# KevynUtopia/Frequency-Aware-Inverse-Consistent-OCTA-Super-Resolution

Hardware: AMD Instinct MI355X
Metric: train-step images/sec (G+D fwd+bwd) on 256x256 OCTA (higher is better)
Workload: dtype f32 (tensors and accumulators fp32; the convolutions' operands enter the matrix cores as f16x2 pairs: hi = f16(x 2^k), lo = f16(x 2^k - hi), k from the tensor's largest magnitude; 3 v_mfma_f32_32x32x16_f16 per product) on every map >= 24 wide with >= 16 channels; narrow maps, 1-channel stems / head

## Files before the change

### frequency-aware-inverse-consistent-octa-super-resolution_amd/csrc/common.h

```cpp
#pragma once
#include <hip/hip_runtime.h>
#include <cstdio>
#include <cstdarg>
#include "faoctasr.h"

namespace faoctasr {

char* err_buf();
int fail(int code, const char* fmt, ...);
enum Route { ROUTE_NONE = 0, ROUTE_GATHER_FLAT = 1, ROUTE_PATCH = 2, ROUTE_WINOGRAD = 3, ROUTE_BF16X3 = 4, ROUTE_M1_FWD = 5, ROUTE_NARROW = 6,
             ROUTE_WGRAD_FLAT = 11, ROUTE_WGRAD_PATCH = 12, ROUTE_WGRAD_S1 = 13, ROUTE_M1_WGRAD = 14, ROUTE_WGRAD_X3 = 15, ROUTE_STEM_DGRAD = 7, ROUTE_STEM_WGRAD = 16,
             ROUTE_NARROW_X2 = 8 };
void set_route(int r);
extern thread_local int g_no_split_k;
extern thread_local unsigned* g_out_absmax;
unsigned* take_out_absmax();

void lds_optin(const void* kernel, size_t lds_bytes);

inline int check_launch(const char* what) {
    hipError_t e = hipGetLastError();
    if (e != hipSuccess) return fail(FAOCTASR_EHIP, "%s: %s", what, hipGetErrorString(e));
    return FAOCTASR_OK;
}

__device__ __forceinline__ float act_apply(float v, int act, float slope) {
    switch (act) {
        case FAOCTASR_ACT_RELU: return v > 0.f ? v : 0.f;
        case FAOCTASR_ACT_LRELU: return v > 0.f ? v : v * slope;
        case FAOCTASR_ACT_TANH: return tanhf(v);
        default: return v;
    }
}
__device__ __forceinline__ float act_grad_from_out(float y, int act, float slope) {
    switch (act) {
        case FAOCTASR_ACT_RELU: return y > 0.f ? 1.f : 0.f;
        case FAOCTASR_ACT_LRELU: return y > 0.f ? 1.f : slope;
        case FAOCTASR_ACT_TANH: return 1.f - y * y;
        default: return 1.f;
    }
}

template <class T>
__device__ __forceinline__ T wave_sum(T v) {
#pragma unroll
    for (int o = 32; o > 0; o >>= 1) v += __shfl_xor(v, o, 64);
    return v;
}

template <class T>
__device__ __forceinline__ T block_sum_256(T v, T* red ) {
    v = wave_sum(v);
    __syncthreads();
    if ((threadIdx.x & 63) == 0) red[threadIdx.x >> 6] = v;
    __syncthreads();
    return red[0] + red[1] + red[2] + red[3];
}

__device__ __forceinline__ void block_partial_store_256(float v, float* red , float* part) {
    v = block_sum_256(v, red);
    if (threadIdx.x == 0) part[blockIdx.x] = v;
}

template <class T>
__device__ __forceinline__ double strided_sum_256(const T* __restrict__ p, long n) {
// ... 39 lines not shown
```

### frequency-aware-inverse-consistent-octa-super-resolution_amd/csrc/conv_m1.hip

```cpp
#include "common.h"

namespace faoctasr {

constexpr int M1_TH = 8, M1_TW = 32, M1_KC = 16;

__global__ __launch_bounds__(256) void conv_m1_fwd_kernel(const float* __restrict__ x, const float* __restrict__ w,
                                                          const float* __restrict__ bias, float* __restrict__ y, int N, int C,
                                                          int H, int W, int KH, int KW, int pad, int act, float slope) {
    extern __shared__ __attribute__((aligned(16))) char smem[];
    float* P = reinterpret_cast<float*>(smem);
    const int PH = M1_TH + KH - 1, PW = M1_TW + KW - 1, PHW = PH * PW, T = KH * KW;
    float* Wl = P + M1_KC * PHW;
    const int tid = threadIdx.x;
    const int tiles_x = (W + M1_TW - 1) / M1_TW, tiles_y = (H + M1_TH - 1) / M1_TH;
    const int n = blockIdx.x / (tiles_x * tiles_y);
    const int r = blockIdx.x - n * tiles_x * tiles_y;
    const int y0 = (r / tiles_x) * M1_TH, x0 = (r % tiles_x) * M1_TW;
    const int ty = tid >> 5, tx = tid & 31;
    const long hw = (long)H * W;
    const float* xn = x + (long)n * C * hw;
    constexpr unsigned OOB = 0x7fffffffu;
    const float invPHW = 1.0f / (float)PHW, invPW = 1.0f / (float)PW;
    float acc = 0.f;
    for (int c0 = 0; c0 < C; c0 += M1_KC) {
// ... 73 lines not shown
#pragma unroll 8
                for (int px = 0; px < M1_TW; ++px) acc += D[py * M1_TW + px] * pp[py * PW + px];
        }
    }
    if (mine) atomicAdd(dw + (long)(c0 + cl) * T + t, acc);
}

typedef float m1f4 __attribute__((ext_vector_type(4)));

__device__ __forceinline__ void m1_row6(const float* __restrict__ row, int xq, int W, bool rowok, float (&v)[6]) {
    m1f4 c = {0.f, 0.f, 0.f, 0.f};
    float l = 0.f, r = 0.f;
    if (rowok) {
        c = *reinterpret_cast<const m1f4*>(row + xq);
        if (xq > 0) l = row[xq - 1];
        if (xq + 4 < W) r = row[xq + 4];
    }
    v[0] = l; v[1] = c[0]; v[2] = c[1]; v[3] = c[2]; v[4] = c[3]; v[5] = r;
}

__global__ __launch_bounds__(256) void conv_m1_fwd3_kernel(const float* __restrict__ x, const float* __restrict__ w, const float* __restrict__ bias,
                                                           float* __restrict__ y, int N, int C, int H, int W, int act, float slope) {
    const int wq = W >> 2;
    const long item = (long)blockIdx.x * 256 + threadIdx.x;
    const long total = (long)N * H * wq;
    if (item >= total) return;
    const int xq = (int)(item % wq) * 4;
    const long t = item / wq;
    const int oy = (int)(t % H), n = (int)(t / H);
    const long hw = (long)H * W;
    const float* xn = x + (long)n * C * hw;
    float acc[4] = {0.f, 0.f, 0.f, 0.f};
    for (int c = 0; c < C; ++c) {
        const float* wc = w + c * 9;
        const float* xc = xn + (long)c * hw;
#pragma unroll
        for (int kh = 0; kh < 3; ++kh) {
            const int iy = oy - 1 + kh;
            float v[6];
            m1_row6(xc + (long)iy * W, xq, W, (unsigned)iy < (unsigned)H, v);
#pragma unroll
            for (int kw = 0; kw < 3; ++kw) {
                const float wv = wc[kh * 3 + kw];
#pragma unroll
                for (int p = 0; p < 4; ++p) acc[p] += wv * v[p + kw];
            }
        }
    }
    const float b = bias ? bias[0] : 0.f;
    m1f4 o = {act_apply(acc[0] + b, act, slope), act_apply(acc[1] + b, act, slope), act_apply(acc[2] + b, act, slope), act_apply(acc[3] + b, act, slope)};
    *reinterpret_cast<m1f4*>(y + (long)n * hw + (long)oy * W + xq) = o;
}

constexpr int M1W_CH = 4, M1W_ROWS = 32;
__global__ __launch_bounds__(256) void conv_m1_wgrad3_kernel(const float* __restrict__ x, const float* __restrict__ dy, float* __restrict__ dw, int N,
                                                             int C, int H, int W) {
    const int lane = threadIdx.x & 63, wave = threadIdx.x >> 6;
    const int cgroups = (C + M1W_CH - 1) / M1W_CH, rsegs = (H + M1W_ROWS - 1) / M1W_ROWS;
    const long item = (long)blockIdx.x * 4 + wave;
    if (item >= (long)N * rsegs * cgroups) return;
    const int cg = (int)(item % cgroups);
    const long t = item / cgroups;
    const int rs = (int)(t % rsegs), n = (int)(t / rsegs);
    const int c0 = cg * M1W_CH, r0 = rs * M1W_ROWS, r1 = r0 + M1W_ROWS < H ? r0 + M1W_ROWS : H;
    const long hw = (long)H * W;
    const float* dyn = dy + (long)n * hw;
    float acc[M1W_CH][9];
#pragma unroll
    for (int c = 0; c < M1W_CH; ++c)
#pragma unroll
        for (int k = 0; k < 9; ++k) acc[c][k] = 0.f;
    for (int xq = lane * 4; xq < W; xq += 256) {
        float ring[M1W_CH][3][6];
#pragma unroll
        for (int c = 0; c < M1W_CH; ++c) {
            const bool cok = c0 + c < C;
            const float* xc = x + ((long)n * C + (cok ? c0 + c : 0)) * hw;
            m1_row6(xc + (long)(r0 - 1) * W, xq, W, cok && r0 - 1 >= 0, ring[c][0]);
            m1_row6(xc + (long)r0 * W, xq, W, cok, ring[c][1]);
        }
        for (int oy = r0; oy < r1; ++oy) {
            const m1f4 g = *reinterpret_cast<const m1f4*>(dyn + (long)oy * W + xq);
#pragma unroll
            for (int c = 0; c < M1W_CH; ++c) {
                const bool cok = c0 + c < C;
                const float* xc = x + ((long)n * C + (cok ? c0 + c : 0)) * hw;
                m1_row6(xc + (long)(oy + 1) * W, xq, W, cok && oy + 1 < H, ring[c][2]);
#pragma unroll
                for (int kh = 0; kh < 3; ++kh)
#pragma unroll
                    for (int kw = 0; kw < 3; ++kw)
#pragma unroll
                        for (int p = 0; p < 4; ++p) acc[c][kh * 3 + kw] += g[p] * ring[c][kh][p + kw];
#pragma unroll
                for (int q = 0; q < 6; ++q) { ring[c][0][q] = ring[c][1][q]; ring[c][1][q] = ring[c][2][q]; }
            }
        }
    }
#pragma unroll
    for (int c = 0; c < M1W_CH; ++c)
#pragma unroll
        for (int k = 0; k < 9; ++k) {
            const float s = wave_sum(acc[c][k]);
            if (lane == c * 9 + k && c0 + c < C) atomicAdd(dw + (long)(c0 + c) * 9 + k, s);
        }
}

int launch_conv_m1_fwd(const float* x, const float* w, const float* bias, float* y, int N, int C, int H, int W, int KH, int KW, int pad,
                       int act, float slope, hipStream_t stream) {
    if (KH == 3 && KW == 3 && pad == 1 && (W & 3) == 0 && N > 0 && H > 0) {
        const long total = (long)N * H * (W >> 2);
        hipLaunchKernelGGL(conv_m1_fwd3_kernel, dim3((unsigned)((total + 255) / 256)), dim3(256), 0, stream, x, w, bias, y, N, C, H, W, act, slope);
        return check_launch("conv_m1_fwd3");
    }
    const int PH = M1_TH + KH - 1, PW = M1_TW + KW - 1;
    const size_t lds = ((size_t)M1_KC * PH * PW + (size_t)M1_KC * KH * KW) * 4;
    const long blocks = (long)N * ((W + M1_TW - 1) / M1_TW) * ((H + M1_TH - 1) / M1_TH);
    if (blocks <= 0) return FAOCTASR_OK;
    hipLaunchKernelGGL(conv_m1_fwd_kernel, dim3((unsigned)blocks), dim3(256), lds, stream, x, w, bias, y, N, C, H, W, KH, KW, pad,
                       act, slope);
    return check_launch("conv_m1_fwd");
}

int launch_conv_m1_wgrad(const float* x, const float* dy, float* dw, int N, int C, int H, int W, int KH, int KW, int pad, int accumulate,
                         hipStream_t st) {
    const int T = KH * KW;
    if (!accumulate && hipMemsetAsync(dw, 0, sizeof(float) * (size_t)C * T, st) != hipSuccess) return fail(FAOCTASR_EHIP, "memset dw failed");
    if (KH == 3 && KW == 3 && pad == 1 && (W & 3) == 0 && N > 0 && H > 0) {
        const long items = (long)N * ((H + M1W_ROWS - 1) / M1W_ROWS) * ((C + M1W_CH - 1) / M1W_CH);
        hipLaunchKernelGGL(conv_m1_wgrad3_kernel, dim3((unsigned)((items + 3) / 4)), dim3(256), 0, st, x, dy, dw, N, C, H, W);
        return check_launch("conv_m1_wgrad3");
    }
    const int CCH = 256 / T;
    const int PH = M1_TH + KH - 1, PW = M1_TW + KW - 1;
    const size_t lds = ((size_t)CCH * PH * PW + M1_TH * M1_TW) * 4;
    const int gy = (C + CCH - 1) / CCH;
    const long ntiles = (long)N * ((W + M1_TW - 1) / M1_TW) * ((H + M1_TH - 1) / M1_TH);
    if (ntiles <= 0) return FAOCTASR_OK;
    long gx = 1024 / gy;
    if (gx < 1) gx = 1;
    if (gx > ntiles) gx = ntiles;
    const int tpb = (int)((ntiles + gx - 1) / gx);
    gx = (ntiles + tpb - 1) / tpb;
    auto k = conv_m1_wgrad_kernel;
    lds_optin((const void*)k, lds);
    hipLaunchKernelGGL(k, dim3((unsigned)gx, gy), dim3(256), lds, st, x, dy, dw, N, C, H, W, KH, KW, pad, tpb, CCH);
    return check_launch("conv_m1_wgrad");
}

}
```

### frequency-aware-inverse-consistent-octa-super-resolution_amd/csrc/igemm.hip

```cpp
#include <cstring>

#include "common.h"
#include "igemm_geom.h"

namespace faoctasr {

typedef float f32x16 __attribute__((ext_vector_type(16)));

__device__ __forceinline__ int reflect_idx(int i, int n) {
    i = i < 0 ? -i : i;
    return i >= n ? 2 * n - 2 - i : i;
}

template <int MT>
__global__ __launch_bounds__(256) void igemm_gather_kernel(const float* __restrict__ x, const float* __restrict__ w,
                                                           const float* __restrict__ bias, float* __restrict__ y,
                                                           const IgemmGeom g, const int ksplit) {
    constexpr int NT = 128, KC = 16, LDA = KC + 1;
    constexpr int MI = MT / 64;
    constexpr int NA = MT * KC / 256;
    __shared__ float A_s[MT * LDA];
    __shared__ float B_s[KC * NT];
    __shared__ int taps_s[64];

// ... 616 lines not shown
    g_wgrad_ws_floats = ws ? nfloats : 0;
    return FAOCTASR_OK;
}

long faoctasr_conv_wgrad_workspace_floats(int C, int M, int KH, int KW, int stride) {
    if (C <= 0 || M <= 0 || KH <= 0 || KW <= 0 || stride <= 0) return fail(FAOCTASR_EINVAL, "conv_wgrad_workspace_floats: bad shape");
    if ((C & 63) || (M & 63)) return 0;
    long blocks = (long)(C / 64) * (M / 64);
    if (!(stride == 1 && KH == 3)) blocks *= KH;
    long slices = 256 / blocks;
    slices = slices < 1 ? 1 : slices;
    return slices * (long)C * M * KH * KW;
}

int faoctasr_conv2d_fwd(const float* x, const float* w, const float* bias, float* y, int N, int C, int IH, int IW, int M,
                        int KH, int KW, int stride, int pad, int reflect, int act, float slope, float* wpack, int wpack_state,
                        int precision, faoctasr_stream_t stream) {
    const unsigned* const slot_a = take_scale_a();
    WgradWsScope ws_scope;
    const float* const res = take_residual();
    if (bad_ptr(x, w, y)) return fail(FAOCTASR_EINVAL, "conv2d_fwd: null pointer");
    if (N < 0 || C <= 0 || M <= 0 || stride <= 0 || pad < 0) return fail(FAOCTASR_EINVAL, "conv2d_fwd: bad shape");
    const int OH = (IH + 2 * pad - KH) / stride + 1, OW = (IW + 2 * pad - KW) / stride + 1;
    if (OH <= 0 || OW <= 0) return fail(FAOCTASR_EINVAL, "conv2d_fwd: kernel (%d x %d) larger than padded input (%d x %d)", KH, KW, IH + 2 * pad, IW + 2 * pad);
    if (M == 1 && stride == 1 && !reflect && 2 * pad == KH - 1 && 2 * pad == KW - 1 && KH <= 7 && IW >= 32)
    {
        set_route(ROUTE_M1_FWD);
        const int rc1 = launch_conv_m1_fwd(x, w, bias, y, N, C, IH, IW, KH, KW, pad, act, slope, (hipStream_t)stream);
        if (rc1 || !res) return rc1;
        return faoctasr_axpby(y, res, y, (long)N * M * OH * OW, 1.f, 1.f, stream);
    }
    IgemmGeom g;
    int rc = geom_fwd(g, N, C, IH, IW, M, OH, OW, KH, KW, stride, pad, reflect, (long)C * KH * KW, (long)KH * KW);
    if (rc) return rc;
    return run_gather(x, w, bias, y, g, act, slope, wpack, wpack_state, precision, (hipStream_t)stream, nullptr, slot_a, res);
}

int faoctasr_conv2d_dgrad(const float* dy, const float* w, float* dx, int N, int C, int IH, int IW, int M, int KH, int KW,
                          int stride, int pad, float* wpack, int wpack_state, int precision, faoctasr_stream_t stream) {
    const unsigned* const slot_a = take_scale_a();
    WgradWsScope ws_scope;
    const float* const res = take_residual();
    if (bad_ptr(dy, w, dx)) return fail(FAOCTASR_EINVAL, "conv2d_dgrad: null pointer");
    const int OH = (IH + 2 * pad - KH) / stride + 1, OW = (IW + 2 * pad - KW) / stride + 1;
    if (OH <= 0 || OW <= 0) return fail(FAOCTASR_EINVAL, "conv2d_dgrad: bad shape");
    {
        const int rc = launch_stem_dgrad(dy, w, dx, N, C, IH, IW, M, KH, KW, stride, pad, (hipStream_t)stream);
        if (rc != 0) {
            set_route(ROUTE_STEM_DGRAD);
            if (rc < 0 || !res) return rc < 0 ? rc : FAOCTASR_OK;
            return faoctasr_axpby(dx, res, dx, (long)N * C * IH * IW, 1.f, 1.f, stream);
        }
    }
    IgemmGeom g;
    int rc = geom_transposed(g, N, M, OH, OW, C, IH, IW, KH, KW, stride, pad, (long)KH * KW, (long)C * KH * KW);
    if (rc) return rc;
    return run_gather(dy, w, nullptr, dx, g, FAOCTASR_ACT_NONE, 0.f, wpack, wpack_state, precision, (hipStream_t)stream, nullptr, slot_a, res);
}

int faoctasr_conv2d_wgrad(const float* x, const float* dy, float* dw, int N, int C, int IH, int IW, int M, int KH, int KW,
                          int stride, int pad, int reflect, int accumulate, int precision, faoctasr_stream_t stream) {
    const unsigned *const slot_x = g_scale_a, *const slot_dy = g_scale_b;
    g_scale_a = g_scale_b = nullptr;
    WgradWsScope ws_scope;
    if (bad_ptr(x, dy, dw)) return fail(FAOCTASR_EINVAL, "conv2d_wgrad: null pointer");
    precision &= 0xff;
    if (precision < 0 || precision > 3) return fail(FAOCTASR_EINVAL, "unknown conv precision %d (0 = f32, 1 = f32 direct, 2 = bf16x3, 3 = f16x2)", precision);
    if (precision == 3 && (!slot_x || !slot_dy)) return fail(FAOCTASR_EINVAL, "conv2d_wgrad: precision 3 (f16x2) needs both absmax slots: faoctasr_conv_set_scales");
    const int OH = (IH + 2 * pad - KH) / stride + 1, OW = (IW + 2 * pad - KW) / stride + 1;
    if (OH <= 0 || OW <= 0) return fail(FAOCTASR_EINVAL, "conv2d_wgrad: bad shape");
    if (M == 1 && stride == 1 && !reflect && 2 * pad == KH - 1 && 2 * pad == KW - 1 && KH <= 7 && IW >= 32)
    {
        set_route(ROUTE_M1_WGRAD);
        return launch_conv_m1_wgrad(x, dy, dw, N, C, IH, IW, KH, KW, pad, accumulate, (hipStream_t)stream);
    }
    {
        const int rc = launch_stem_wgrad(x, dy, dw, N, C, IH, IW, M, KH, KW, stride, pad, reflect, accumulate, (hipStream_t)stream);
        if (rc != 0) { set_route(ROUTE_STEM_WGRAD); return rc < 0 ? rc : FAOCTASR_OK; }
    }
    IgemmGeom g;
    int rc = geom_fwd(g, N, C, IH, IW, M, OH, OW, KH, KW, stride, pad, reflect, (long)C * KH * KW, (long)KH * KW);
    if (rc) return rc;
    if (OW >= 24) {
        if (!accumulate && hipMemsetAsync(dw, 0, sizeof(float) * (size_t)M * C * KH * KW, (hipStream_t)stream) != hipSuccess)
            return fail(FAOCTASR_EHIP, "memset dw failed");
        if (precision >= 2) {
            rc = launch_wgrad_x3(x, dy, dw, N, C, IH, IW, M, OH, OW, KH, KW, stride, pad, reflect, (long)C * KH * KW, (long)KH * KW,
                                 (hipStream_t)stream, precision == 3, slot_x, slot_dy);
            if (rc != 0) { set_route(ROUTE_WGRAD_X3); return rc < 0 ? rc : FAOCTASR_OK; }
        }
        rc = launch_wgrad_s1(x, dy, dw, N, C, IH, IW, M, OH, OW, KH, KW, stride, pad, reflect, (long)C * KH * KW, (long)KH * KW,
                             (hipStream_t)stream);
        if (rc != 0) { set_route(ROUTE_WGRAD_S1); return rc < 0 ? rc : FAOCTASR_OK; }
        rc = launch_wgrad_patch(x, dy, dw, N, C, IH, IW, M, OH, OW, KH, KW, stride, pad, reflect, (long)C * KH * KW, (long)KH * KW,
                                (hipStream_t)stream);
        if (rc != 0) { set_route(ROUTE_WGRAD_PATCH); return rc < 0 ? rc : FAOCTASR_OK; }
        set_route(ROUTE_WGRAD_FLAT);
        return launch_wgrad(x, dy, dw, g, (long)M * C * KH * KW, 1, (hipStream_t)stream);
    }
    set_route(ROUTE_WGRAD_FLAT);
    return launch_wgrad(x, dy, dw, g, (long)M * C * KH * KW, accumulate, (hipStream_t)stream);
}

int faoctasr_conv_transpose2d_fwd(const float* x, const float* w, const float* bias, float* y, int N, int C, int IH, int IW,
                                  int M, int KH, int KW, int stride, int pad, int out_pad, int act, float slope, float* wpack,
                                  int wpack_state, int precision, faoctasr_stream_t stream) {
// ... 61 lines not shown
```

### frequency-aware-inverse-consistent-octa-super-resolution_amd/csrc/igemm_geom.h

```cpp
#pragma once
#include <hip/hip_runtime.h>

namespace faoctasr {

constexpr int PATCH_MAX_PER_THREAD = 20;

struct IgemmGeom {
    int N, C, IH, IW;
    int M, OH, OW;
    int SI, SO;
    int nphase;
    int reflect;
    int act;
    float slope;
    long wsm, wsc;
    int ph_py[4], ph_px[4], ph_gh[4], ph_gw[4], ph_t0[5];
    int taps[64];
};

struct PatchGeom {
    int N, C, IH, IW, M, OH, OW, SI, SO, nphase, reflect, act;
    float slope;
    int Mpad;
    long wsm, wsc;
// ... 39 lines not shown
struct PackJob {
    long block0;
    long total;
    const float* w;
    float* wp;
    int type, blocks;
    union {
        PatchGeom patch;
        WinoGeom wino;
        SplitGeom split;
    } g;
};
constexpr int PACK_JOB_BYTES = 1024;
static_assert(sizeof(PackJob) <= PACK_JOB_BYTES, "PackJob outgrew its slot");
inline int pack_job_blocks(long rows) { return (int)(rows > 1024 ? 1024 : rows); }

int patch_geom_from(const IgemmGeom& f, PatchGeom& g);
long patch_pack_floats(const PatchGeom& g);
int launch_pack(const float* w, float* wp, const PatchGeom& g, hipStream_t s);
int launch_patch(const float* x, const float* wp, const float* bias, float* y, PatchGeom& g, int act, float slope, hipStream_t s);
int launch_narrow(const float* x, const float* wp, const float* bias, float* y, PatchGeom& g, int act, float slope, hipStream_t s);
int launch_wgrad_patch(const float* x, const float* dy, float* dw, int N, int C, int IH, int IW, int M, int OH, int OW, int KH, int KW,
                       int stride, int pad, int reflect, long wsm, long wsc, hipStream_t s);
int launch_wgrad_x3(const float* x, const float* dy, float* dw, int N, int C, int IH, int IW, int M, int OH, int OW, int KH, int KW,
                    int stride, int pad, int reflect, long wsm, long wsc, hipStream_t s, int f16 = 0, const unsigned* x_slot = nullptr,
                    const unsigned* dy_slot = nullptr);
int launch_wgrad_s1(const float* x, const float* dy, float* dw, int N, int C, int IH, int IW, int M, int OH, int OW, int KH, int KW,
                    int stride, int pad, int reflect, long wsm, long wsc, hipStream_t s);

int split_try(const IgemmGeom& f, const float* x, const float* w, const float* bias, float* y, int act, float slope, float* wpack,
              int wpack_state, hipStream_t s, PackJob* sink = nullptr, int f16 = 0, const unsigned* x_slot = nullptr,
              const float* res = nullptr);
long split_pack_floats_for(const IgemmGeom& f, bool narrow = false);
int narrow_x2_try(const IgemmGeom& f, const float* x, const float* w, const float* bias, float* y, int act, float slope, float* wpack,
                  int wpack_state, hipStream_t s, PackJob* sink, const unsigned* x_slot, const float* res, float* ws, long ws_floats);
long narrow_x2_workspace_floats_for(const IgemmGeom& f);
int narrow_x2_eligible(const SplitGeom& g);
long narrow_x2_workspace_floats(const SplitGeom& g);
int launch_narrow_x2(const float* x, const float* wp, const float* bias, float* y, SplitGeom& g, int act, float slope, hipStream_t s,
                     const unsigned* x_slot, const float* res, float* ws, long ws_floats);
extern thread_local const unsigned* g_scale_a;
extern thread_local const unsigned* g_scale_b;
extern thread_local float* g_wgrad_ws;
extern thread_local long g_wgrad_ws_floats;

int wino_try(const IgemmGeom& f, const float* x, const float* w, const float* bias, float* y, int act, float slope, float* wpack,
             int wpack_state, hipStream_t s, PackJob* sink = nullptr);
long wino_pack_floats_for(const IgemmGeom& f);

int launch_conv_m1_fwd(const float* x, const float* w, const float* bias, float* y, int N, int C, int H, int W, int KH, int KW, int pad,
                       int act, float slope, hipStream_t stream);
int launch_conv_m1_wgrad(const float* x, const float* dy, float* dw, int N, int C, int H, int W, int KH, int KW, int pad, int accumulate,
                         hipStream_t st);

bool stem_dgrad_eligible(int C, int IH, int IW, int M, int KH, int KW, int stride, int pad);
bool stem_wgrad_eligible(int C, int IH, int IW, int KH, int KW, int stride, int pad, int reflect);
extern thread_local bool g_wgrad_dry_run;
int launch_stem_dgrad(const float* dy, const float* w, float* dx, int N, int C, int IH, int IW, int M, int KH, int KW, int stride, int pad,
                      hipStream_t s);
int launch_stem_wgrad(const float* x, const float* dy, float* dw, int N, int C, int IH, int IW, int M, int KH, int KW, int stride, int pad,
                      int reflect, int accumulate, hipStream_t s);

}
```

### frequency-aware-inverse-consistent-octa-super-resolution_amd/csrc/pointwise.hip

```cpp
#include <mutex>
#include <unordered_map>
#include "common.h"
#include "split16.h"

namespace faoctasr {

thread_local char g_err[512] = "";
char* err_buf() { return g_err; }
int get_route();
int fail(int code, const char* fmt, ...) {
    va_list ap;
    va_start(ap, fmt);
    vsnprintf(g_err, sizeof(g_err), fmt, ap);
    va_end(ap);
    return code;
}

thread_local int g_route = 0;
thread_local unsigned* g_out_absmax = nullptr;
unsigned* take_out_absmax() {
    unsigned* p = g_out_absmax;
    g_out_absmax = nullptr;
    return p;
}
// ... 110 lines not shown
    const long stride = (long)gridDim.x * blockDim.x;
    for (long i = (long)blockIdx.x * blockDim.x + threadIdx.x; i < n; i += stride) y[i] = alpha * a[i] + beta * b[i];
}

__global__ void fill_kernel(float* __restrict__ p, long n, float v) {
    const long stride = (long)gridDim.x * blockDim.x;
    for (long i = (long)blockIdx.x * blockDim.x + threadIdx.x; i < n; i += stride) p[i] = v;
}

__global__ __launch_bounds__(256) void channel_sum_kernel(const float* __restrict__ dy, float* __restrict__ db, int N, int C, int HW,
                                                          long per) {
    __shared__ float red[4];
    const int c = blockIdx.y;
    const long L = (long)N * HW;
    long e0 = (long)blockIdx.x * per, e1 = e0 + per;
    e1 = e1 < L ? e1 : L;
    float s = 0.f;
    if ((HW & 3) == 0) {
        for (long e = e0 + 4L * threadIdx.x; e < e1; e += 1024) {
            const long n = e / HW;
            const float4 v = *reinterpret_cast<const float4*>(dy + ((long)n * C + c) * HW + (e - n * HW));
            s += v.x + v.y + v.z + v.w;
        }
    } else {
        for (long e = e0 + threadIdx.x; e < e1; e += 256) {
            const long n = e / HW;
            s += dy[((long)n * C + c) * HW + (e - n * HW)];
        }
    }
    s = block_sum_256(s, red);
    if (threadIdx.x == 0) atomicAdd(db + c, s);
}

__global__ void reflect_pad_bwd_kernel(const float* __restrict__ dxp, float* __restrict__ dx, long NC, int H, int W, int p) {
    const long tot = NC * H * W;
    const int HP = H + 2 * p, WP = W + 2 * p;
    const long stride = (long)gridDim.x * blockDim.x;
    for (long i = (long)blockIdx.x * blockDim.x + threadIdx.x; i < tot; i += stride) {
        const long nc = i / ((long)H * W);
        const int r = (int)(i - nc * H * W);
        const int yy = r / W, xx = r - yy * W;
        int ry[3], rx[3], ny = 0, nx = 0;
        ry[ny++] = yy + p;
        if (yy >= 1 && yy <= p) ry[ny++] = p - yy;
        if (yy <= H - 2 && yy >= H - 1 - p) ry[ny++] = 2 * (H - 1) - yy + p;
        rx[nx++] = xx + p;
        if (xx >= 1 && xx <= p) rx[nx++] = p - xx;
        if (xx <= W - 2 && xx >= W - 1 - p) rx[nx++] = 2 * (W - 1) - xx + p;
        float s = 0.f;
        for (int a = 0; a < ny; ++a)
            for (int b = 0; b < nx; ++b) s += dxp[(nc * HP + ry[a]) * WP + rx[b]];
        dx[i] = s;
    }
}

__global__ void haar_fwd_kernel(const float* __restrict__ x, float* __restrict__ ll, float* __restrict__ hi, long NC, int H, int W) {
    const int h = H >> 1, w = W >> 1;
    const long tot = NC * h * w;
    const long stride = (long)gridDim.x * blockDim.x;
    for (long i = (long)blockIdx.x * blockDim.x + threadIdx.x; i < tot; i += stride) {
        const long nc = i / ((long)h * w);
        const int r = (int)(i - nc * h * w);
        const int yy = r / w, xx = r - yy * w;
        const float* p = x + (nc * H + 2 * yy) * W + 2 * xx;
        const float2 t = *reinterpret_cast<const float2*>(p);
        const float2 u = *reinterpret_cast<const float2*>(p + W);
        const float a = t.x, b = t.y, c = u.x, d = u.y;
        if (ll) ll[i] = (a + b + c + d) * 0.5f;
        if (hi) {
            float* q = hi + (nc * 3) * h * w + r;
            q[0] = (a + b - c - d) * 0.5f;
            q[(long)h * w] = (a - b + c - d) * 0.5f;
            q[2L * h * w] = (a - b - c + d) * 0.5f;
        }
    }
}

__global__ void haar_inv_kernel(const float* __restrict__ ll, const float* __restrict__ hi, float* __restrict__ x, long NC, int H, int W) {
    const int h = H >> 1, w = W >> 1;
    const long tot = NC * h * w;
    const long stride = (long)gridDim.x * blockDim.x;
    for (long i = (long)blockIdx.x * blockDim.x + threadIdx.x; i < tot; i += stride) {
        const long nc = i / ((long)h * w);
        const int r = (int)(i - nc * h * w);
        const int yy = r / w, xx = r - yy * w;
        const float l = ll ? ll[i] : 0.f;
        float lh = 0.f, hl = 0.f, hh = 0.f;
        if (hi) {
            const float* q = hi + (nc * 3) * h * w + r;
            lh = q[0]; hl = q[(long)h * w]; hh = q[2L * h * w];
        }
        float* p = x + (nc * H + 2 * yy) * W + 2 * xx;
        *reinterpret_cast<float2*>(p) = make_float2((l + lh + hl + hh) * 0.5f, (l + lh - hl - hh) * 0.5f);
        *reinterpret_cast<float2*>(p + W) = make_float2((l - lh + hl - hh) * 0.5f, (l - lh - hl + hh) * 0.5f);
    }
}

__global__ void haar_dfront_fwd_kernel(const float* __restrict__ x, float* __restrict__ y, int N, int H, int W, int mode) {
    const int h = H >> 1, w = W >> 1;
    const long tot = (long)N * h * w;
    const long stride = (long)gridDim.x * blockDim.x;
    for (long i = (long)blockIdx.x * blockDim.x + threadIdx.x; i < tot; i += stride) {
        const long n = i / ((long)h * w);
        const int r = (int)(i - n * h * w);
        const int yy = r / w, xx = r - yy * w;
        const float* p = x + (n * H + 2 * yy) * W + 2 * xx;
// ... 286 lines not shown
    if (tot <= 0) return FAOCTASR_OK;
    hipLaunchKernelGGL(cat2_act_fwd_kernel, dim3(grid_for(tot, 256)), dim3(256), 0, (hipStream_t)stream, a, b, y, N, (long)Ca * HW,
                       (long)Cb * HW, act, slope, faoctasr::take_out_absmax());
    return check_launch("cat2_act_fwd");
}

int faoctasr_cat2_act_bwd(const float* dy, const float* y, float* da, float* db, int N, int Ca, int Cb, int HW, int act, float slope,
                          faoctasr_stream_t stream) {
    if (!dy) return fail(FAOCTASR_EINVAL, "cat2_act_bwd: null pointer");
    if (act != FAOCTASR_ACT_NONE && !y) return fail(FAOCTASR_EINVAL, "cat2_act_bwd: mask needs y");
    const long tot = (long)N * (Ca + Cb) * HW;
    if (tot <= 0) return FAOCTASR_OK;
    hipLaunchKernelGGL(cat2_act_bwd_kernel, dim3(grid_for(tot, 256)), dim3(256), 0, (hipStream_t)stream, dy, y, da, db, N,
                       (long)Ca * HW, (long)Cb * HW, act, slope);
    return check_launch("cat2_act_bwd");
}

int faoctasr_axpby(const float* a, const float* b, float* y, long n, float alpha, float beta, faoctasr_stream_t stream) {
    if (!a || !b || !y) return fail(FAOCTASR_EINVAL, "axpby: null pointer");
    if (n <= 0) return FAOCTASR_OK;
    hipLaunchKernelGGL(axpby_kernel, dim3(grid_for(n, 256)), dim3(256), 0, (hipStream_t)stream, a, b, y, n, alpha, beta);
    return check_launch("axpby");
}

int faoctasr_fill(float* p, long n, float value, faoctasr_stream_t stream) {
    if (!p) return fail(FAOCTASR_EINVAL, "fill: null pointer");
    if (n <= 0) return FAOCTASR_OK;
    hipLaunchKernelGGL(fill_kernel, dim3(grid_for(n, 256)), dim3(256), 0, (hipStream_t)stream, p, n, value);
    return check_launch("fill");
}

int faoctasr_channel_sum(const float* dy, float* db, int N, int C, int HW, int accumulate, faoctasr_stream_t stream) {
    if (!dy || !db) return fail(FAOCTASR_EINVAL, "channel_sum: null pointer");
    if (C <= 0) return FAOCTASR_OK;
    hipStream_t st = (hipStream_t)stream;
    if (!accumulate && hipMemsetAsync(db, 0, sizeof(float) * C, st) != hipSuccess) return fail(FAOCTASR_EHIP, "channel_sum: memset failed");
    const long L = (long)N * HW;
    long S = (1024 + C - 1) / C;
    const long maxs = (L + 4095) / 4096;
    S = S < maxs ? S : maxs;
    S = S < 1 ? 1 : S;
    long per = (L + S - 1) / S;
    per = (per + 3) & ~3L;
    S = (L + per - 1) / per;
    hipLaunchKernelGGL(channel_sum_kernel, dim3((unsigned)S, C), dim3(256), 0, st, dy, db, N, C, HW, per);
    return check_launch("channel_sum");
}

int faoctasr_reflect_pad_bwd(const float* dxp, float* dx, int NC, int H, int W, int p, faoctasr_stream_t stream) {
    if (!dxp || !dx) return fail(FAOCTASR_EINVAL, "reflect_pad_bwd: null pointer");
    if (p >= H || p >= W) return fail(FAOCTASR_EINVAL, "reflect_pad_bwd: pad >= size");
    const long tot = (long)NC * H * W;
    if (tot <= 0) return FAOCTASR_OK;
    hipLaunchKernelGGL(reflect_pad_bwd_kernel, dim3(grid_for(tot, 256)), dim3(256), 0, (hipStream_t)stream, dxp, dx, (long)NC, H, W, p);
    return check_launch("reflect_pad_bwd");
}

int faoctasr_haar_dwt2d_fwd(const float* x, float* ll, float* hi, long NC, int H, int W, faoctasr_stream_t stream) {
    if (!x) return fail(FAOCTASR_EINVAL, "haar_dwt2d_fwd: null pointer");
    if ((H & 1) || (W & 1)) return fail(FAOCTASR_EUNSUPPORTED, "haar_dwt2d: odd size %dx%d (reference path uses even sizes only)", H, W);
    const long tot = NC * (H / 2) * (W / 2);
    if (tot <= 0) return FAOCTASR_OK;
    hipLaunchKernelGGL(haar_fwd_kernel, dim3(grid_for(tot, 256)), dim3(256), 0, (hipStream_t)stream, x, ll, hi, NC, H, W);
    return check_launch("haar_fwd");
}

int faoctasr_haar_dwt2d_bwd(const float* dll, const float* dhi, float* dx, long NC, int H, int W, faoctasr_stream_t stream) {
    if (!dx) return fail(FAOCTASR_EINVAL, "haar_dwt2d_bwd: null pointer");
    if ((H & 1) || (W & 1)) return fail(FAOCTASR_EUNSUPPORTED, "haar_dwt2d: odd size %dx%d", H, W);
    const long tot = NC * (H / 2) * (W / 2);
    if (tot <= 0) return FAOCTASR_OK;
    hipLaunchKernelGGL(haar_inv_kernel, dim3(grid_for(tot, 256)), dim3(256), 0, (hipStream_t)stream, dll, dhi, dx, NC, H, W);
    return check_launch("haar_inv");
}

int faoctasr_haar_dfront_fwd(const float* x, float* y, int N, int H, int W, int mode, faoctasr_stream_t stream) {
    if (!x || !y) return fail(FAOCTASR_EINVAL, "haar_dfront_fwd: null pointer");
    if ((H & 1) || (W & 1)) return fail(FAOCTASR_EUNSUPPORTED, "haar_dfront: odd size");
    const long tot = (long)N * (H / 2) * (W / 2);
    if (tot <= 0) return FAOCTASR_OK;
    hipLaunchKernelGGL(haar_dfront_fwd_kernel, dim3(grid_for(tot, 256)), dim3(256), 0, (hipStream_t)stream, x, y, N, H, W, mode);
    return check_launch("haar_dfront_fwd");
}

int faoctasr_haar_dfront_bwd(const float* dy, float* dx, int N, int H, int W, int mode, faoctasr_stream_t stream) {
    if (!dy || !dx) return fail(FAOCTASR_EINVAL, "haar_dfront_bwd: null pointer");
    if ((H & 1) || (W & 1)) return fail(FAOCTASR_EUNSUPPORTED, "haar_dfront: odd size");
    const long tot = (long)N * (H / 2) * (W / 2);
    if (tot <= 0) return FAOCTASR_OK;
    hipLaunchKernelGGL(haar_dfront_bwd_kernel, dim3(grid_for(tot, 256)), dim3(256), 0, (hipStream_t)stream, dy, dx, N, H, W, mode);
    return check_launch("haar_dfront_bwd");
}

int faoctasr_freq_mix_fwd(const float* x, const float* low_hp, const float* low_lp, float* hf, float* lf, long n,
                          faoctasr_stream_t stream) {
    if (!x || !low_hp || !low_lp || !hf || !lf) return fail(FAOCTASR_EINVAL, "freq_mix_fwd: null pointer");
    if (n <= 0) return FAOCTASR_OK;
    hipLaunchKernelGGL(freq_mix_fwd_kernel, dim3(grid_for(n, 256)), dim3(256), 0, (hipStream_t)stream, x, low_hp, low_lp, hf, lf, n);
    return check_launch("freq_mix_fwd");
}

int faoctasr_freq_mix_bwd(const float* x, const float* low_hp, const float* low_lp, const float* g_hf, const float* g_lf, float* s_hp,
                          float* s_lp, float* dx_direct, long n, faoctasr_stream_t stream) {
    if (!x || !low_hp || !low_lp || !s_hp || !s_lp || !dx_direct) return fail(FAOCTASR_EINVAL, "freq_mix_bwd: null pointer");
    if (n <= 0) return FAOCTASR_OK;
    hipLaunchKernelGGL(freq_mix_bwd_kernel, dim3(grid_for(n, 256)), dim3(256), 0, (hipStream_t)stream, x, low_hp, low_lp, g_hf, g_lf,
// ... 85 lines not shown
```

Before: 138.3.

## Add direct M=1 3x3 dgrad, strip-based wgrad with DPP shifts, vectorised reflect-pad backward

Adds a dedicated dgrad kernel for single-output-channel 3x3 convolutions that computes dx directly per channel group, optionally fusing the residual add, instead of going through the implicit-GEMM path. Rewrites the M=1 wgrad kernel into strip tiles that use DPP lane shifts for halo columns, prefetch the next rows, and reduce through DPP and shared memory before a single atomic per weight. Adds a float4 reflect-pad backward kernel. These target launch overhead, narrow GEMM inefficiency and scalar memory traffic in small backward ops, at the cost of more specialised code paths.

After: 139.1 (median of 6 runs). No clear change (+0.6%).

```diff
diff --git a/frequency-aware-inverse-consistent-octa-super-resolution_amd/csrc/common.h b/frequency-aware-inverse-consistent-octa-super-resolution_amd/csrc/common.h
--- a/frequency-aware-inverse-consistent-octa-super-resolution_amd/csrc/common.h
+++ b/frequency-aware-inverse-consistent-octa-super-resolution_amd/csrc/common.h
@@ -10,7 +10,7 @@
 int fail(int code, const char* fmt, ...);
 enum Route { ROUTE_NONE = 0, ROUTE_GATHER_FLAT = 1, ROUTE_PATCH = 2, ROUTE_WINOGRAD = 3, ROUTE_BF16X3 = 4, ROUTE_M1_FWD = 5, ROUTE_NARROW = 6,
              ROUTE_WGRAD_FLAT = 11, ROUTE_WGRAD_PATCH = 12, ROUTE_WGRAD_S1 = 13, ROUTE_M1_WGRAD = 14, ROUTE_WGRAD_X3 = 15, ROUTE_STEM_DGRAD = 7, ROUTE_STEM_WGRAD = 16,
-             ROUTE_NARROW_X2 = 8 };
+             ROUTE_NARROW_X2 = 8, ROUTE_M1_DGRAD = 9 };
 void set_route(int r);
 extern thread_local int g_no_split_k;
 extern thread_local unsigned* g_out_absmax;
diff --git a/frequency-aware-inverse-consistent-octa-super-resolution_amd/csrc/conv_m1.hip b/frequency-aware-inverse-consistent-octa-super-resolution_amd/csrc/conv_m1.hip
--- a/frequency-aware-inverse-consistent-octa-super-resolution_amd/csrc/conv_m1.hip
+++ b/frequency-aware-inverse-consistent-octa-super-resolution_amd/csrc/conv_m1.hip
@@ -149,17 +149,58 @@
     *reinterpret_cast<m1f4*>(y + (long)n * hw + (long)oy * W + xq) = o;
 }
 
-constexpr int M1W_CH = 4, M1W_ROWS = 32;
-__global__ __launch_bounds__(256) void conv_m1_wgrad3_kernel(const float* __restrict__ x, const float* __restrict__ dy, float* __restrict__ dw, int N,
-                                                             int C, int H, int W) {
-    const int lane = threadIdx.x & 63, wave = threadIdx.x >> 6;
-    const int cgroups = (C + M1W_CH - 1) / M1W_CH, rsegs = (H + M1W_ROWS - 1) / M1W_ROWS;
-    const long item = (long)blockIdx.x * 4 + wave;
-    if (item >= (long)N * rsegs * cgroups) return;
-    const int cg = (int)(item % cgroups);
-    const long t = item / cgroups;
-    const int rs = (int)(t % rsegs), n = (int)(t / rsegs);
-    const int c0 = cg * M1W_CH, r0 = rs * M1W_ROWS, r1 = r0 + M1W_ROWS < H ? r0 + M1W_ROWS : H;
+constexpr int M1W_CH = 4;
+
+__device__ __forceinline__ float m1_from_lane_below(float v) {
+    return __int_as_float(__builtin_amdgcn_update_dpp(0, __float_as_int(v), 0x138, 0xf, 0xf, true));
+}
+__device__ __forceinline__ float m1_from_lane_above(float v) {
+    return __int_as_float(__builtin_amdgcn_update_dpp(0, __float_as_int(v), 0x130, 0xf, 0xf, true));
+}
+
+__device__ __forceinline__ m1f4 m1_load4(const float* __restrict__ plane, int iy, int H, int W, int xq, bool colok) {
+    const int cy = iy < 0 ? 0 : (iy < H ? iy : H - 1);
+    return *reinterpret_cast<const m1f4*>(plane + (long)cy * W + (colok ? xq : 0));
+}
+template <bool MULTI>
+__device__ __forceinline__ void m1_finish6(m1f4 c, const float* __restrict__ plane, int iy, int H, int W, int xq, bool colok, int lane, float (&v)[6]) {
+    const bool ok = colok && (unsigned)iy < (unsigned)H;
+    if (!ok) c = m1f4{0.f, 0.f, 0.f, 0.f};
+    float l = m1_from_lane_below(c[3]), r = m1_from_lane_above(c[0]);
+    if (MULTI) {
+        const float* row = plane + (long)iy * W;
+        if (lane == 0 && ok && xq > 0) l = row[xq - 1];
+        if (lane == 63 && ok && xq + 4 < W) r = row[xq + 4];
+    }
+    v[0] = l; v[1] = c[0]; v[2] = c[1]; v[3] = c[2]; v[4] = c[3]; v[5] = r;
+}
+
+constexpr int M1SW_ROWS = 8;
+template <int CTRL, int ROW_MASK>
+__device__ __forceinline__ float m1_dpp_add(float v) {
+    return v + __int_as_float(__builtin_amdgcn_update_dpp(0, __float_as_int(v), CTRL, ROW_MASK, 0xf, true));
+}
+__device__ __forceinline__ float m1_wave_sum_to_lane63(float v) {
+    v = m1_dpp_add<0x111, 0xf>(v);
+    v = m1_dpp_add<0x112, 0xf>(v);
+    v = m1_dpp_add<0x114, 0xf>(v);
+    v = m1_dpp_add<0x118, 0xf>(v);
+    v = m1_dpp_add<0x142, 0xa>(v);
+    v = m1_dpp_add<0x143, 0xc>(v);
+    return v;
+}
+
+template <bool MULTI>
+__global__ __launch_bounds__(256) void conv_m1_wgrad3_strip_kernel(const float* __restrict__ x, const float* __restrict__ dy, float* __restrict__ dw,
+                                                                   int N, int C, int H, int W) {
+    __shared__ float red[4][M1W_CH * 9];
+    const int lane = threadIdx.x & 63, wave = __builtin_amdgcn_readfirstlane(threadIdx.x >> 6);
+    const int cgroups = (C + M1W_CH - 1) / M1W_CH, rblocks = (H + 4 * M1SW_ROWS - 1) / (4 * M1SW_ROWS);
+    unsigned b = blockIdx.x;
+    const int c0 = (int)(b % (unsigned)cgroups) * M1W_CH; b /= (unsigned)cgroups;
+    const int rb = (int)(b % (unsigned)rblocks);
+    const int n = (int)(b / (unsigned)rblocks);
+    const int r0 = (rb * 4 + wave) * M1SW_ROWS, r1 = r0 + M1SW_ROWS < H ? r0 + M1SW_ROWS : H;
     const long hw = (long)H * W;
     const float* dyn = dy + (long)n * hw;
     float acc[M1W_CH][9];
@@ -167,40 +208,101 @@
     for (int c = 0; c < M1W_CH; ++c)
 #pragma unroll
         for (int k = 0; k < 9; ++k) acc[c][k] = 0.f;
-    for (int xq = lane * 4; xq < W; xq += 256) {
-        float ring[M1W_CH][3][6];
-#pragma unroll
-        for (int c = 0; c < M1W_CH; ++c) {
-            const bool cok = c0 + c < C;
-            const float* xc = x + ((long)n * C + (cok ? c0 + c : 0)) * hw;
-            m1_row6(xc + (long)(r0 - 1) * W, xq, W, cok && r0 - 1 >= 0, ring[c][0]);
-            m1_row6(xc + (long)r0 * W, xq, W, cok, ring[c][1]);
-        }
-        for (int oy = r0; oy < r1; ++oy) {
-            const m1f4 g = *reinterpret_cast<const m1f4*>(dyn + (long)oy * W + xq);
+    if (r0 < H) {
+        for (int x0 = 0; x0 < W; x0 += 256) {
+            const int xq = x0 + lane * 4;
+            const bool colok = xq < W;
+            const float* xc[M1W_CH];
+            bool cok[M1W_CH];
 #pragma unroll
             for (int c = 0; c < M1W_CH; ++c) {
-                const bool cok = c0 + c < C;
-                const float* xc = x + ((long)n * C + (cok ? c0 + c : 0)) * hw;
-                m1_row6(xc + (long)(oy + 1) * W, xq, W, cok && oy + 1 < H, ring[c][2]);
-#pragma unroll
-                for (int kh = 0; kh < 3; ++kh)
-#pragma unroll
-                    for (int kw = 0; kw < 3; ++kw)
-#pragma unroll
-                        for (int p = 0; p < 4; ++p) acc[c][kh * 3 + kw] += g[p] * ring[c][kh][p + kw];
-#pragma unroll
-                for (int q = 0; q < 6; ++q) { ring[c][0][q] = ring[c][1][q]; ring[c][1][q] = ring[c][2][q]; }
+                cok[c] = colok && c0 + c < C;
+                xc[c] = x + ((long)n * C + (c0 + c < C ? c0 + c : 0)) * hw;
             }
+            float ring[M1W_CH][3][6];
+            m1f4 raw[M1W_CH][3];
+#pragma unroll
+            for (int c = 0; c < M1W_CH; ++c)
+#pragma unroll
+                for (int j = 0; j < 3; ++j) raw[c][j] = m1_load4(xc[c], r0 - 1 + j, H, W, xq, colok);
+            m1f4 g = *reinterpret_cast<const m1f4*>(dyn + (long)r0 * W + (colok ? xq : 0));
+#pragma unroll
+            for (int c = 0; c < M1W_CH; ++c)
+#pragma unroll
+                for (int j = 0; j < 3; ++j) m1_finish6<MULTI>(raw[c][j], xc[c], r0 - 1 + j, H, W, xq, cok[c], lane, ring[c][j]);
+#pragma unroll 1
+            for (int oy = r0; oy < r1; ++oy) {
+                const int ny = oy + 2 <= r1 ? oy + 2 : r1, gy = oy + 1 < r1 ? oy + 1 : oy;
+                m1f4 nx[M1W_CH];
+#pragma unroll
+                for (int c = 0; c < M1W_CH; ++c) nx[c] = m1_load4(xc[c], ny, H, W, xq, colok);
+                const m1f4 gn = *reinterpret_cast<const m1f4*>(dyn + (long)gy * W + (colok ? xq : 0));
+                if (!colok) g = m1f4{0.f, 0.f, 0.f, 0.f};
+#pragma unroll
+                for (int c = 0; c < M1W_CH; ++c)
+#pragma unroll
+                    for (int kh = 0; kh < 3; ++kh)
+#pragma unroll
+                        for (int kw = 0; kw < 3; ++kw)
+#pragma unroll
+                            for (int p = 0; p < 4; ++p) acc[c][kh * 3 + kw] += g[p] * ring[c][kh][p + kw];
+#pragma unroll
+                for (int c = 0; c < M1W_CH; ++c) {
+#pragma unroll
+                    for (int q = 0; q < 6; ++q) { ring[c][0][q] = ring[c][1][q]; ring[c][1][q] = ring[c][2][q]; }
+                    m1_finish6<MULTI>(nx[c], xc[c], ny, H, W, xq, cok[c], lane, ring[c][2]);
+                }
+                g = gn;
+            }
         }
     }
 #pragma unroll
     for (int c = 0; c < M1W_CH; ++c)
 #pragma unroll
         for (int k = 0; k < 9; ++k) {
-            const float s = wave_sum(acc[c][k]);
-            if (lane == c * 9 + k && c0 + c < C) atomicAdd(dw + (long)(c0 + c) * 9 + k, s);
-        }
+            const float s = m1_wave_sum_to_lane63(acc[c][k]);
+            if (lane == 63) red[wave][c * 9 + k] = s;
+        }
+    __syncthreads();
+    const int i = threadIdx.x;
+    if (i < M1W_CH * 9 && c0 + i / 9 < C) atomicAdd(dw + (long)c0 * 9 + i, ((red[0][i] + red[1][i]) + red[2][i]) + red[3][i]);
+}
+
+constexpr int M1D_CG = 16;
+template <bool RES>
+__global__ __launch_bounds__(256) void conv_m1_dgrad3_kernel(const float* __restrict__ dy, const float* __restrict__ w, const float* __restrict__ res,
+                                                             float* __restrict__ dx, int N, int C, int H, int W) {
+    const int wq = W >> 2;
+    const long item = (long)blockIdx.x * 256 + threadIdx.x;
+    if (item >= (long)N * H * wq) return;
+    const int xq = (int)(item % wq) * 4;
+    const long t = item / wq;
+    const int oy = (int)(t % H), n = (int)(t / H);
+    const long hw = (long)H * W;
+    const float* dyn = dy + (long)n * hw;
+    float v[3][6];
+#pragma unroll
+    for (int j = 0; j < 3; ++j) {
+        const int iy = oy - 1 + j;
+        m1_row6(dyn + (long)iy * W, xq, W, (unsigned)iy < (unsigned)H, v[j]);
+    }
+    const int c0 = blockIdx.y * M1D_CG, c1 = c0 + M1D_CG < C ? c0 + M1D_CG : C;
+    const long o0 = (long)n * C * hw + (long)oy * W + xq;
+#pragma unroll 4
+    for (int c = c0; c < c1; ++c) {
+        const float* wc = w + c * 9;
+        m1f4 o = {0.f, 0.f, 0.f, 0.f};
+        if (RES) o = *reinterpret_cast<const m1f4*>(res + o0 + (long)c * hw);
+#pragma unroll
+        for (int kh = 0; kh < 3; ++kh)
+#pragma unroll
+            for (int kw = 0; kw < 3; ++kw) {
+                const float wv = wc[kh * 3 + kw];
+#pragma unroll
+                for (int p = 0; p < 4; ++p) o[p] += wv * v[2 - kh][p + 2 - kw];
+            }
+        *reinterpret_cast<m1f4*>(dx + o0 + (long)c * hw) = o;
+    }
 }
 
 int launch_conv_m1_fwd(const float* x, const float* w, const float* bias, float* y, int N, int C, int H, int W, int KH, int KW, int pad,
@@ -224,9 +326,12 @@
     const int T = KH * KW;
     if (!accumulate && hipMemsetAsync(dw, 0, sizeof(float) * (size_t)C * T, st) != hipSuccess) return fail(FAOCTASR_EHIP, "memset dw failed");
     if (KH == 3 && KW == 3 && pad == 1 && (W & 3) == 0 && N > 0 && H > 0) {
-        const long items = (long)N * ((H + M1W_ROWS - 1) / M1W_ROWS) * ((C + M1W_CH - 1) / M1W_CH);
-        hipLaunchKernelGGL(conv_m1_wgrad3_kernel, dim3((unsigned)((items + 3) / 4)), dim3(256), 0, st, x, dy, dw, N, C, H, W);
-        return check_launch("conv_m1_wgrad3");
+        const long blocks = (long)N * ((H + 4 * M1SW_ROWS - 1) / (4 * M1SW_ROWS)) * ((C + M1W_CH - 1) / M1W_CH);
+        if (blocks <= 0x7fffffffL) {
+            if (W > 256) hipLaunchKernelGGL(conv_m1_wgrad3_strip_kernel<true>, dim3((unsigned)blocks), dim3(256), 0, st, x, dy, dw, N, C, H, W);
+            else hipLaunchKernelGGL(conv_m1_wgrad3_strip_kernel<false>, dim3((unsigned)blocks), dim3(256), 0, st, x, dy, dw, N, C, H, W);
+            return check_launch("conv_m1_wgrad3_strip");
+        }
     }
     const int CCH = 256 / T;
     const int PH = M1_TH + KH - 1, PW = M1_TW + KW - 1;
@@ -245,4 +350,20 @@
     return check_launch("conv_m1_wgrad");
 }
 
-}
+static bool m1_dgrad_eligible(int C, int IH, int IW, int M, int KH, int KW, int stride, int pad) {
+    return M == 1 && KH == 3 && KW == 3 && stride == 1 && pad == 1 && (IW & 3) == 0 && IH > 0 && IW > 0 && C <= 65535 * M1D_CG;
+}
+
+int launch_conv_m1_dgrad(const float* dy, const float* w, const float* res, float* dx, int N, int C, int IH, int IW, int M, int KH, int KW,
+                         int stride, int pad, hipStream_t st) {
+    if (!m1_dgrad_eligible(C, IH, IW, M, KH, KW, stride, pad)) return 0;
+    if (N <= 0) return 1;
+    const long gx = ((long)N * IH * (IW >> 2) + 255) / 256, gy = (C + M1D_CG - 1) / M1D_CG;
+    if (gx > 0x7fffffffL) return fail(FAOCTASR_EINVAL, "conv_m1_dgrad: grid too large");
+    if (res) hipLaunchKernelGGL(conv_m1_dgrad3_kernel<true>, dim3((unsigned)gx, (unsigned)gy), dim3(256), 0, st, dy, w, res, dx, N, C, IH, IW);
+    else hipLaunchKernelGGL(conv_m1_dgrad3_kernel<false>, dim3((unsigned)gx, (unsigned)gy), dim3(256), 0, st, dy, w, res, dx, N, C, IH, IW);
+    const int rc = check_launch("conv_m1_dgrad3");
+    return rc == FAOCTASR_OK ? 1 : rc;
+}
+
+}
diff --git a/frequency-aware-inverse-consistent-octa-super-resolution_amd/csrc/igemm.hip b/frequency-aware-inverse-consistent-octa-super-resolution_amd/csrc/igemm.hip
--- a/frequency-aware-inverse-consistent-octa-super-resolution_amd/csrc/igemm.hip
+++ b/frequency-aware-inverse-consistent-octa-super-resolution_amd/csrc/igemm.hip
@@ -692,6 +692,10 @@
             return faoctasr_axpby(dx, res, dx, (long)N * C * IH * IW, 1.f, 1.f, stream);
         }
     }
+    if (wpack_state != 1) {
+        const int rc = launch_conv_m1_dgrad(dy, w, res, dx, N, C, IH, IW, M, KH, KW, stride, pad, (hipStream_t)stream);
+        if (rc != 0) { set_route(ROUTE_M1_DGRAD); return rc < 0 ? rc : FAOCTASR_OK; }
+    }
     IgemmGeom g;
     int rc = geom_transposed(g, N, M, OH, OW, C, IH, IW, KH, KW, stride, pad, (long)KH * KW, (long)C * KH * KW);
     if (rc) return rc;
diff --git a/frequency-aware-inverse-consistent-octa-super-resolution_amd/csrc/igemm_geom.h b/frequency-aware-inverse-consistent-octa-super-resolution_amd/csrc/igemm_geom.h
--- a/frequency-aware-inverse-consistent-octa-super-resolution_amd/csrc/igemm_geom.h
+++ b/frequency-aware-inverse-consistent-octa-super-resolution_amd/csrc/igemm_geom.h
@@ -115,6 +115,8 @@
                        int act, float slope, hipStream_t stream);
 int launch_conv_m1_wgrad(const float* x, const float* dy, float* dw, int N, int C, int H, int W, int KH, int KW, int pad, int accumulate,
                          hipStream_t st);
+int launch_conv_m1_dgrad(const float* dy, const float* w, const float* res, float* dx, int N, int C, int IH, int IW, int M, int KH, int KW,
+                         int stride, int pad, hipStream_t st);
 
 bool stem_dgrad_eligible(int C, int IH, int IW, int M, int KH, int KW, int stride, int pad);
 bool stem_wgrad_eligible(int C, int IH, int IW, int KH, int KW, int stride, int pad, int reflect);
diff --git a/frequency-aware-inverse-consistent-octa-super-resolution_amd/csrc/pointwise.hip b/frequency-aware-inverse-consistent-octa-super-resolution_amd/csrc/pointwise.hip
--- a/frequency-aware-inverse-consistent-octa-super-resolution_amd/csrc/pointwise.hip
+++ b/frequency-aware-inverse-consistent-octa-super-resolution_amd/csrc/pointwise.hip
@@ -186,6 +186,43 @@
             for (int b = 0; b < nx; ++b) s += dxp[(nc * HP + ry[a]) * WP + rx[b]];
         dx[i] = s;
     }
+}
+
+typedef float fold_f4 __attribute__((ext_vector_type(4)));
+typedef float fold_f4u __attribute__((ext_vector_type(4), aligned(4)));
+
+__global__ __launch_bounds__(256) void reflect_pad_bwd_quad_kernel(const float* __restrict__ dxp, float* __restrict__ dx, int H, int W, int p) {
+    const int wq = W >> 2;
+    const int item = blockIdx.x * 256 + threadIdx.x;
+    if (item >= H * wq) return;
+    const int yy = item / wq, xq = (item - yy * wq) * 4;
+    const int HP = H + 2 * p, WP = W + 2 * p;
+    const long nc = blockIdx.y;
+    int ry[3], ny = 0;
+    ry[ny++] = yy + p;
+    if (yy >= 1 && yy <= p) ry[ny++] = p - yy;
+    if (yy <= H - 2 && yy >= H - 1 - p) ry[ny++] = 2 * (H - 1) - yy + p;
+    const bool left = xq <= p, right = xq + 3 >= W - 1 - p;
+    fold_f4 s = {0.f, 0.f, 0.f, 0.f};
+    for (int a = 0; a < ny; ++a) {
+        const float* row = dxp + (nc * HP + ry[a]) * WP;
+        s += *reinterpret_cast<const fold_f4u*>(row + xq + p);
+        if (left) {
+#pragma unroll
+            for (int q = 0; q < 4; ++q) {
+                const int xx = xq + q;
+                if (xx >= 1 && xx <= p) s[q] += row[p - xx];
+            }
+        }
+        if (right) {
+#pragma unroll
+            for (int q = 0; q < 4; ++q) {
+                const int xx = xq + q;
+                if (xx <= W - 2 && xx >= W - 1 - p) s[q] += row[2 * (W - 1) - xx + p];
+            }
+        }
+    }
+    *reinterpret_cast<fold_f4*>(dx + (nc * H + yy) * W + xq) = s;
 }
 
 __global__ void haar_fwd_kernel(const float* __restrict__ x, float* __restrict__ ll, float* __restrict__ hi, long NC, int H, int W) {
@@ -578,6 +615,11 @@
     if (p >= H || p >= W) return fail(FAOCTASR_EINVAL, "reflect_pad_bwd: pad >= size");
     const long tot = (long)NC * H * W;
     if (tot <= 0) return FAOCTASR_OK;
+    if ((W & 3) == 0 && 2 * p < W && NC <= 65535 && (long)H * W < (1L << 31) && (reinterpret_cast<uintptr_t>(dx) & 15) == 0) {
+        const unsigned gx = (unsigned)(((long)H * (W >> 2) + 255) / 256);
+        hipLaunchKernelGGL(reflect_pad_bwd_quad_kernel, dim3(gx, (unsigned)NC), dim3(256), 0, (hipStream_t)stream, dxp, dx, H, W, p);
+        return check_launch("reflect_pad_bwd_quad");
+    }
     hipLaunchKernelGGL(reflect_pad_bwd_kernel, dim3(grid_for(tot, 256)), dim3(256), 0, (hipStream_t)stream, dxp, dx, (long)NC, H, W, p);
     return check_launch("reflect_pad_bwd");
 }
```
